# Zeudon/sound-event-localization-detection

Hardware: AMD Instinct MI355X
Metric: training clips/sec (4ch FOA 60s@24kHz) (higher is better)
Workload: dtype bf16; 1 GPU; crnn FOA 4-ch 60s clips, bs=32 windows (BASELINE configs[1]); parallelism=dp1

## Files before the change

sound-event-localization-detection_amd/csrc/conv3x3_image.h:

```cpp
#pragma once

#include <hip/hip_runtime.h>

namespace seld {
namespace conv3x3 {

typedef __attribute__((ext_vector_type(8))) __bf16 bf16x8;
typedef __attribute__((ext_vector_type(4))) short s16x4;
typedef __attribute__((ext_vector_type(8))) short s16x8;
typedef __attribute__((ext_vector_type(4))) float f32x4;
typedef __attribute__((address_space(3))) s16x4 lds_s16x4;

constexpr int kThreads = 256;
constexpr int kChannels = 64;
constexpr int kPitch = 80;

template <int F, int P>
struct Image {
  static_assert(F == 8 || F == 16 || F == 32, "frequency bins: 8, 16 or 32");
  static_assert(P % F == 0, "a chunk is whole time rows");
  static constexpr int TC = P / F;
  static constexpr int kRows = (TC + 2) * (F + 2);
  static constexpr int kLoads = (kRows * 8 + kThreads - 1) / kThreads;
};

template <int F>
__device__ __forceinline__ int image_row(int pos) {
  return (pos / F + 1) * (F + 2) + pos % F + 1;
}

template <int F>
__device__ __forceinline__ constexpr int tap_shift(int tap) {
  return (tap / 3 - 1) * (F + 2) + (tap % 3 - 1);
}

template <int F, int P>
__device__ __forceinline__ uint4 image_piece(const unsigned short* __restrict__ src, long clip_row, int t0, int T,
                                             int C, int c0, int piece) {
  const int r = piece >> 3, ch = piece & 7;
  const int tr = r / (F + 2), f = r - tr * (F + 2) - 1, t = t0 - 1 + tr;
  uint4 v = make_uint4(0u, 0u, 0u, 0u);
  if (r < Image<F, P>::kRows && t >= 0 && t < T && f >= 0 && f < F)
    v = *reinterpret_cast<const uint4*>(src + ((clip_row + t) * F + f) * C + c0 + ch * 8);
  return v;
}

__device__ __forceinline__ s16x4 tr_read(const unsigned short* base, int offset_shorts) {
  return __builtin_amdgcn_ds_read_tr16_b64_v4i16((lds_s16x4*)(base + offset_shorts));
}

__device__ __forceinline__ bf16x8 join(s16x4 lo, s16x4 hi) {
  const s16x8 v = __builtin_shufflevector(lo, hi, 0, 1, 2, 3, 4, 5, 6, 7);
  return __builtin_bit_cast(bf16x8, v);
}

}
}
```

sound-event-localization-detection_amd/csrc/conv3x3_loop.h:

```cpp
#pragma once

#include <hip/hip_bf16.h>

#include "conv3x3_image.h"

namespace seld {
namespace conv3x3 {

constexpr int kLoopP = 256;
constexpr int kLoopKc = kChannels;

template <int F, int NT, bool kFwd>
struct LoopGeom {
  static_assert(NT == 64 || NT == 128, "result channels per workgroup: 64 or 128");
  using Img = Image<F, kLoopP>;
  static constexpr int kWPitch = kFwd ? kPitch : NT + 16;
  static constexpr int kWRows = kFwd ? NT : kLoopKc;
  static constexpr int kWLoads = kLoopKc * NT / 8 / kThreads;
  static constexpr int kNTiles = NT / 32;
  static constexpr int kImgBatch = (Img::kLoads + 1) / 2;
  static constexpr int kImgShorts = Img::kRows * kPitch;
  static constexpr int kLdsShorts = kImgShorts + kWRows * kWPitch;
  static_assert(2 * kLdsShorts * 2 <= 160 * 1024, "two workgroups per CU");
};

template <int kCtrl>
__device__ __forceinline__ float dpp_add(float v) {
  return v + __builtin_bit_cast(float, __builtin_amdgcn_update_dpp(0, __builtin_bit_cast(int, v), kCtrl, 0xf, 0xf, false));
}
__device__ __forceinline__ float row16_sum(float v) {
  v = dpp_add<0xB1>(v);
  v = dpp_add<0x4E>(v);
  v = dpp_add<0x141>(v);
  return dpp_add<0x140>(v);
}

template <int F, int NT, bool kFwd, bool kStats>
__device__ __forceinline__ void conv3x3_loop(const unsigned short* __restrict__ src, const unsigned short* __restrict__ w,
                                             int T, int Cn, int Ck, int chunks_per_clip,
                                             unsigned short* __restrict__ dst, float* __restrict__ partials) {
  static_assert(kFwd || !kStats, "the statistics epilogue belongs to the forward direction");
  using G = LoopGeom<F, NT, kFwd>;
  __shared__ __attribute__((aligned(16))) unsigned short lds[G::kLdsShorts];
  unsigned short* const limg = lds;
  unsigned short* const lw = lds + G::kImgShorts;

  const int tid = threadIdx.x, lane = tid & 63, wave = tid >> 6;
  const int wm = wave >> 1, wn = wave & 1;
  const int chunk = blockIdx.x, n0 = blockIdx.y * NT;
  const int b = chunk / chunks_per_clip, t0 = (chunk - b * chunks_per_clip) * G::Img::TC;
  const long clip_row = static_cast<long>(b) * T;

  f32x4 acc[8][G::kNTiles];
#pragma unroll
  for (int m = 0; m < 8; ++m)
#pragma unroll
    for (int n = 0; n < G::kNTiles; ++n) acc[m][n] = f32x4{0.0f, 0.0f, 0.0f, 0.0f};

  const int g = lane >> 4, q = (lane >> 2) & 3, p = lane & 3, l15 = lane & 15;
  const int w_off = kFwd ? (wn * (NT / 2) + l15) * G::kWPitch + 8 * g
                         : (4 * g + q) * G::kWPitch + wn * (NT / 2) + 4 * p;
  const int d_off = image_row<F>(wm * 128 + l15) * kPitch + 8 * g;
  auto d_rows = [](int m) { return image_row<F>(16 * m) - image_row<F>(0); };

  static_assert(G::kWLoads == 2 || G::kWLoads == 4, "weight pieces per thread");
  uint4 rw0, rw1, rw2 = make_uint4(0u, 0u, 0u, 0u), rw3 = rw2;
  auto w_piece = [&](int stage, int i) {
    const int kc = stage / 9, tap = stage - kc * 9;
    const int piece = tid + i * kThreads;
    if constexpr (kFwd) {
      const int row = piece >> 3, ch = piece & 7;
      return *reinterpret_cast<const uint4*>(w + (static_cast<long>(n0 + row) * 9 + tap) * Ck + kc * kLoopKc + ch * 8);
    } else {
      const int row = piece / (NT / 8), ch = piece % (NT / 8);
      return *reinterpret_cast<const uint4*>(w + (static_cast<long>(kc * kLoopKc + row) * 9 + tap) * Cn + n0 + ch * 8);
    }
  };
  auto load_w = [&](int stage) {
    rw0 = w_piece(stage, 0);
    rw1 = w_piece(stage, 1);
    if constexpr (G::kWLoads == 4) {
      rw2 = w_piece(stage, 2);
      rw3 = w_piece(stage, 3);
    }
  };
  auto w_slot = [&](int i) {
    const int piece = tid + i * kThreads;
    if constexpr (kFwd) return reinterpret_cast<uint4*>(lw + (piece >> 3) * G::kWPitch + (piece & 7) * 8);
    else return reinterpret_cast<uint4*>(lw + piece / (NT / 8) * G::kWPitch + piece % (NT / 8) * 8);
  };

  const int stages = Ck / kLoopKc * 9;
  load_w(0);
  for (int stage = 0; stage < stages; ++stage) {
    const int kc = stage / 9, tap = stage - kc * 9;
    uint4 rimg[G::kImgBatch];
    auto load_img = [&](int first) {
#pragma unroll
      for (int i = 0; i < G::kImgBatch; ++i)
        rimg[i] = image_piece<F, kLoopP>(src, clip_row, t0, T, Ck, kc * kLoopKc, tid + (first + i) * kThreads);
    };
    auto store_img = [&](int first) {
#pragma unroll
      for (int i = 0; i < G::kImgBatch; ++i) {
        const int piece = tid + (first + i) * kThreads, ch = piece & 7;
        if constexpr (kFwd) {
          if (piece < G::Img::kRows * 8) *reinterpret_cast<uint4*>(limg + (piece >> 3) * kPitch + ch * 8) = rimg[i];
        } else {
          unsigned short* const slot = limg + (piece >> 3) * kPitch + (ch >> 2) * 32 + 16 * (ch & 1) + 4 * ((ch >> 1) & 1);
          if (piece < G::Img::kRows * 8) {
            *reinterpret_cast<uint2*>(slot) = make_uint2(rimg[i].x, rimg[i].y);
            *reinterpret_cast<uint2*>(slot + 8) = make_uint2(rimg[i].z, rimg[i].w);
          }
        }
      }
    };
    if (tap == 0) load_img(0);
    __syncthreads();
    *w_slot(0) = rw0;
    *w_slot(1) = rw1;
    if constexpr (G::kWLoads == 4) {
      *w_slot(2) = rw2;
      *w_slot(3) = rw3;
    }
    if (tap == 0) {
      store_img(0);
      load_img(G::kImgBatch);
      store_img(G::kImgBatch);
    }
    __syncthreads();
    load_w(min(stage + 1, stages - 1));

    const int shift = (kFwd ? tap_shift<F>(tap) : -tap_shift<F>(tap)) * kPitch;
#pragma unroll
    for (int ks = 0; ks < kLoopKc / 32; ++ks) {
      bf16x8 wf[G::kNTiles];
#pragma unroll
      for (int n = 0; n < G::kNTiles; ++n) {
        if constexpr (kFwd)
          wf[n] = *reinterpret_cast<const bf16x8*>(lw + w_off + n * 16 * G::kWPitch + ks * 32);
        else
          wf[n] = join(tr_read(lw, w_off + ks * 32 * G::kWPitch + n * 16),
                       tr_read(lw, w_off + (ks * 32 + 16) * G::kWPitch + n * 16));
      }
#pragma unroll
      for (int m = 0; m < 8; ++m) {
        const bf16x8 df = *reinterpret_cast<const bf16x8*>(limg + d_off + d_rows(m) * kPitch + shift + ks * 32);
#pragma unroll
        for (int n = 0; n < G::kNTiles; ++n)
          acc[m][n] = __builtin_amdgcn_mfma_f32_16x16x32_bf16(wf[n], df, acc[m][n], 0, 0, 0);
      }
    }
  }

  const int rows_left = (T - t0) * F;
  unsigned short* const out = dst + ((clip_row + t0) * F) * Cn + n0 + wn * (NT / 2) + 4 * g;
#pragma unroll
  for (int m = 0; m < 8; ++m) {
    const int pos = wm * 128 + m * 16 + l15;
    if (pos >= rows_left) continue;
#pragma unroll
    for (int n = 0; n < G::kNTiles; ++n) {
      const f32x4 v = acc[m][n];
      const unsigned lo = static_cast<unsigned>(__bfloat16_as_ushort(__float2bfloat16(v[0]))) |
                          (static_cast<unsigned>(__bfloat16_as_ushort(__float2bfloat16(v[1]))) << 16);
      const unsigned hi = static_cast<unsigned>(__bfloat16_as_ushort(__float2bfloat16(v[2]))) |
                          (static_cast<unsigned>(__bfloat16_as_ushort(__float2bfloat16(v[3]))) << 16);
      *reinterpret_cast<uint2*>(out + static_cast<long>(pos) * Cn + n * 16) = make_uint2(lo, hi);
    }
  }

  if constexpr (kStats) {
    float* const red = reinterpret_cast<float*>(lds);
    __syncthreads();
#pragma unroll
    for (int n = 0; n < G::kNTiles; ++n)
#pragma unroll
      for (int j = 0; j < 4; ++j) {
        float r[8], s[8];
#pragma unroll
        for (int m = 0; m < 8; ++m) {
          const float v = __uint_as_float(static_cast<unsigned>(__bfloat16_as_ushort(__float2bfloat16(acc[m][n][j]))) << 16);
          r[m] = wm * 128 + m * 16 + l15 < rows_left ? v : 0.0f;
          s[m] = r[m] * r[m];
        }
        const float s1 = row16_sum(((r[0] + r[1]) + (r[2] + r[3])) + ((r[4] + r[5]) + (r[6] + r[7])));
        const float s2 = row16_sum(((s[0] + s[1]) + (s[2] + s[3])) + ((s[4] + s[5]) + (s[6] + s[7])));
        if (l15 == 0) {
          const int c = wn * (NT / 2) + n * 16 + 4 * g + j;
          red[(wm * 2 + 0) * NT + c] = s1;
          red[(wm * 2 + 1) * NT + c] = s2;
        }
      }
    __syncthreads();
    if (tid < 2 * NT) {
      const int stat = tid / NT, c = tid - stat * NT;
      partials[(static_cast<long>(stat) * gridDim.x + chunk) * Cn + n0 + c] = red[stat * NT + c] + red[(2 + stat) * NT + c];
    }
  }
}

}
}
```

sound-event-localization-detection_amd/csrc/convdgrad.hip:

```cpp
#include <hip/hip_bf16.h>

#include "conv3x3_loop.h"
#include "seld_common.h"

namespace seld {

namespace {

using namespace conv3x3;

constexpr int kDgP = kLoopP;
constexpr int kDgKc = kLoopKc;

template <int F, int NT>
__global__ __launch_bounds__(kThreads, 2) void conv3x3_dgrad_kernel(
    const unsigned short* __restrict__ dy, const unsigned short* __restrict__ w, int T, int Cin, int Cout,
    int chunks_per_clip, unsigned short* __restrict__ dx) {
  conv3x3_loop<F, NT, false, false>(dy, w, T, Cin, Cout, chunks_per_clip, dx, nullptr);
}

bool dgrad_supported(int64_t F, int64_t Cin, int64_t Cout) {
  return (F == 8 || F == 16 || F == 32) && Cin > 0 && Cout > 0 && Cin % 64 == 0 && Cout % kDgKc == 0;
}

template <int F>
void launch_dgrad(const unsigned short* dy, const unsigned short* w, int B, int T, int Cin, int Cout,
                  unsigned short* dx, hipStream_t stream) {
  constexpr int tc = kDgP / F;
  const int chunks_per_clip = (T + tc - 1) / tc;
  const unsigned chunks = static_cast<unsigned>(B * chunks_per_clip);
  if (Cin % 128 == 0)
    hipLaunchKernelGGL((conv3x3_dgrad_kernel<F, 128>), dim3(chunks, static_cast<unsigned>(Cin / 128)), dim3(kThreads),
                       0, stream, dy, w, T, Cin, Cout, chunks_per_clip, dx);
  else
    hipLaunchKernelGGL((conv3x3_dgrad_kernel<F, 64>), dim3(chunks, static_cast<unsigned>(Cin / 64)), dim3(kThreads), 0,
                       stream, dy, w, T, Cin, Cout, chunks_per_clip, dx);
}

}

}

extern "C" {

int seld_conv3x3_dgrad_supported(int64_t F, int64_t Cin, int64_t Cout) {
  return seld::dgrad_supported(F, Cin, Cout) ? 1 : 0;
}

int seld_conv3x3_dgrad(const void* dy, const void* w, int64_t B, int64_t T, int64_t F, int64_t Cin, int64_t Cout,
                       void* dx, void* stream_) {
  using namespace seld;
  const DeviceState* st = current_state();
  if (!st) return kErrNotInitialised;
  if (!dy || !w || !dx || B <= 0 || T <= 0) return fail(kErrInvalidArgument, "seld_conv3x3_dgrad: bad argument");
  if (!dgrad_supported(F, Cin, Cout))
    return fail(kErrUnsupported, "seld_conv3x3_dgrad: F in {8, 16, 32} and channel counts % 64 == 0 required");
  if (B * ((T + kDgP / F - 1) / (kDgP / F)) > 0x7fffffffLL || B * T > 0x7fffffffLL)
    return fail(kErrUnsupported, "seld_conv3x3_dgrad: too many positions");
  if (((reinterpret_cast<uintptr_t>(dy) | reinterpret_cast<uintptr_t>(w) | reinterpret_cast<uintptr_t>(dx)) & 15) != 0)
    return fail(kErrInvalidArgument, "seld_conv3x3_dgrad: 16-byte aligned tensors required");
  hipStream_t stream = static_cast<hipStream_t>(stream_);
  const unsigned short* ds = static_cast<const unsigned short*>(dy);
  const unsigned short* ws = static_cast<const unsigned short*>(w);
  unsigned short* xs = static_cast<unsigned short*>(dx);
  const int b = static_cast<int>(B), t = static_cast<int>(T), ci = static_cast<int>(Cin), co = static_cast<int>(Cout);
  switch (F) {
    case 8: launch_dgrad<8>(ds, ws, b, t, ci, co, xs, stream); break;
    case 16: launch_dgrad<16>(ds, ws, b, t, ci, co, xs, stream); break;
    default: launch_dgrad<32>(ds, ws, b, t, ci, co, xs, stream); break;
  }
  SELD_HIP_TRY(hipGetLastError());
  return kOk;
}

}
```

sound-event-localization-detection_amd/csrc/convfwd.hip:

```cpp
#include <hip/hip_bf16.h>

#include "conv3x3_loop.h"
#include "seld_common.h"

namespace seld {

namespace {

using namespace conv3x3;

template <int F, int NT, bool kStats>
__global__ __launch_bounds__(kThreads, 2) void conv3x3_fwd_kernel(
    const unsigned short* __restrict__ x, const unsigned short* __restrict__ w, int T, int Cin, int Cout,
    int chunks_per_clip, unsigned short* __restrict__ y, float* __restrict__ partials) {
  conv3x3_loop<F, NT, true, kStats>(x, w, T, Cout, Cin, chunks_per_clip, y, partials);
}

bool fwd_supported(int64_t F, int64_t Cin, int64_t Cout) {
  return (F == 8 || F == 16 || F == 32) && Cin > 0 && Cout > 0 && Cin % kLoopKc == 0 && Cout % 64 == 0;
}

int64_t fwd_chunks(int64_t B, int64_t T, int64_t F) {
  const int64_t tc = kLoopP / F;
  return B * ((T + tc - 1) / tc);
}

template <int F, int NT>
void launch_fwd_tile(const unsigned short* x, const unsigned short* w, int T, int Cin, int Cout, int chunks_per_clip,
                     unsigned chunks, unsigned short* y, float* partials, hipStream_t stream) {
  const dim3 grid(chunks, static_cast<unsigned>(Cout / NT));
  if (partials)
    hipLaunchKernelGGL((conv3x3_fwd_kernel<F, NT, true>), grid, dim3(kThreads), 0, stream, x, w, T, Cin, Cout,
                       chunks_per_clip, y, partials);
  else
    hipLaunchKernelGGL((conv3x3_fwd_kernel<F, NT, false>), grid, dim3(kThreads), 0, stream, x, w, T, Cin, Cout,
                       chunks_per_clip, y, partials);
}

template <int F>
void launch_fwd(const unsigned short* x, const unsigned short* w, int B, int T, int Cin, int Cout, unsigned short* y,
                float* partials, hipStream_t stream) {
  constexpr int tc = kLoopP / F;
  const int chunks_per_clip = (T + tc - 1) / tc;
  const unsigned chunks = static_cast<unsigned>(B * chunks_per_clip);
  if (Cout % 128 == 0) launch_fwd_tile<F, 128>(x, w, T, Cin, Cout, chunks_per_clip, chunks, y, partials, stream);
  else launch_fwd_tile<F, 64>(x, w, T, Cin, Cout, chunks_per_clip, chunks, y, partials, stream);
}

}

}

extern "C" {

int seld_conv3x3_forward_supported(int64_t F, int64_t Cin, int64_t Cout) {
  return seld::fwd_supported(F, Cin, Cout) ? 1 : 0;
}

int64_t seld_conv3x3_forward_chunks(int64_t B, int64_t T, int64_t F) {
  if (!(F == 8 || F == 16 || F == 32) || B <= 0 || T <= 0) return 0;
  return seld::fwd_chunks(B, T, F);
}

int seld_conv3x3_forward(const void* x, const void* w, int64_t B, int64_t T, int64_t F, int64_t Cin, int64_t Cout,
                         void* y, float* partials, void* stream_) {
  using namespace seld;
  const DeviceState* st = current_state();
  if (!st) return kErrNotInitialised;
  if (!x || !w || !y || B <= 0 || T <= 0) return fail(kErrInvalidArgument, "seld_conv3x3_forward: bad argument");
  if (!fwd_supported(F, Cin, Cout))
    return fail(kErrUnsupported, "seld_conv3x3_forward: F in {8, 16, 32} and channel counts % 64 == 0 required");
  if (fwd_chunks(B, T, F) > 0x7fffffffLL || B * T > 0x7fffffffLL)
    return fail(kErrUnsupported, "seld_conv3x3_forward: too many positions");
  if (((reinterpret_cast<uintptr_t>(x) | reinterpret_cast<uintptr_t>(w) | reinterpret_cast<uintptr_t>(y)) & 15) != 0)
    return fail(kErrInvalidArgument, "seld_conv3x3_forward: 16-byte aligned tensors required");
  hipStream_t stream = static_cast<hipStream_t>(stream_);
  const unsigned short* xs = static_cast<const unsigned short*>(x);
  const unsigned short* ws = static_cast<const unsigned short*>(w);
  unsigned short* ys = static_cast<unsigned short*>(y);
  const int b = static_cast<int>(B), t = static_cast<int>(T), ci = static_cast<int>(Cin), co = static_cast<int>(Cout);
  switch (F) {
    case 8: launch_fwd<8>(xs, ws, b, t, ci, co, ys, partials, stream); break;
    case 16: launch_fwd<16>(xs, ws, b, t, ci, co, ys, partials, stream); break;
    default: launch_fwd<32>(xs, ws, b, t, ci, co, ys, partials, stream); break;
  }
  SELD_HIP_TRY(hipGetLastError());
  return kOk;
}

}
```

Before: 172.0 clips/s.

## Software-pipeline LDS reads in conv3x3 loop and widen output stores

Restructures the inner MFMA loop of the shared conv3x3 forward and dgrad kernel into a flat step sequence with a rotating lookahead buffer of image fragments and staggered weight fragment reads. Scheduling barriers pin the order so LDS latency overlaps MFMA work. Weight loads now use a precomputed 32-bit per-thread offset off a per-stage base pointer, and the channel limit guard added to the support checks keeps that offset from overflowing. The epilogue uses permlane16_swap to pair rows and emit 16-byte stores instead of 8-byte ones. In exchange, register pressure rises and the scheduler has less freedom.

```diff
diff --git a/sound-event-localization-detection_amd/csrc/conv3x3_image.h b/sound-event-localization-detection_amd/csrc/conv3x3_image.h
--- a/sound-event-localization-detection_amd/csrc/conv3x3_image.h
+++ b/sound-event-localization-detection_amd/csrc/conv3x3_image.h
@@ -9,6 +9,8 @@
 typedef __attribute__((ext_vector_type(4))) short s16x4;
 typedef __attribute__((ext_vector_type(8))) short s16x8;
 typedef __attribute__((ext_vector_type(4))) float f32x4;
+typedef __attribute__((ext_vector_type(4))) unsigned u32x4;
+typedef __attribute__((ext_vector_type(2))) unsigned u32x2;
 typedef __attribute__((address_space(3))) s16x4 lds_s16x4;
 
 constexpr int kThreads = 256;
diff --git a/sound-event-localization-detection_amd/csrc/conv3x3_loop.h b/sound-event-localization-detection_amd/csrc/conv3x3_loop.h
--- a/sound-event-localization-detection_amd/csrc/conv3x3_loop.h
+++ b/sound-event-localization-detection_amd/csrc/conv3x3_loop.h
@@ -9,6 +9,7 @@
 
 constexpr int kLoopP = 256;
 constexpr int kLoopKc = kChannels;
+constexpr int kLoopMaxChannels = 1 << 20;
 
 template <int F, int NT, bool kFwd>
 struct LoopGeom {
@@ -19,6 +20,7 @@
   static constexpr int kWLoads = kLoopKc * NT / 8 / kThreads;
   static constexpr int kNTiles = NT / 32;
   static constexpr int kImgBatch = (Img::kLoads + 1) / 2;
+  static constexpr int kAhead = NT == 128 ? 2 : 4;
   static constexpr int kImgShorts = Img::kRows * kPitch;
   static constexpr int kLdsShorts = kImgShorts + kWRows * kWPitch;
   static_assert(2 * kLdsShorts * 2 <= 160 * 1024, "two workgroups per CU");
@@ -64,30 +66,31 @@
   auto d_rows = [](int m) { return image_row<F>(16 * m) - image_row<F>(0); };
 
   static_assert(G::kWLoads == 2 || G::kWLoads == 4, "weight pieces per thread");
-  uint4 rw0, rw1, rw2 = make_uint4(0u, 0u, 0u, 0u), rw3 = rw2;
-  auto w_piece = [&](int stage, int i) {
+  constexpr int kWPieceRows = kFwd ? kThreads / 8 : kThreads / (NT / 8);
+  const long w_row = 9L * (kFwd ? Ck : Cn);
+  const unsigned w_voff = kFwd ? ((tid >> 3) * 9 * Ck + (tid & 7) * 8) * 2u
+                               : ((tid / (NT / 8)) * 9 * Cn + (tid % (NT / 8)) * 8) * 2u;
+  u32x4 rw0, rw1, rw2 = u32x4{0u, 0u, 0u, 0u}, rw3 = rw2;
+  auto w_piece = [&](const unsigned short* base, int i, unsigned voff) {
+    return *reinterpret_cast<const u32x4*>(reinterpret_cast<const char*>(base + i * kWPieceRows * w_row) + voff);
+  };
+  auto load_w = [&](int stage) {
+    unsigned voff = w_voff;
+    asm volatile("" : "+v"(voff));
     const int kc = stage / 9, tap = stage - kc * 9;
-    const int piece = tid + i * kThreads;
-    if constexpr (kFwd) {
-      const int row = piece >> 3, ch = piece & 7;
-      return *reinterpret_cast<const uint4*>(w + (static_cast<long>(n0 + row) * 9 + tap) * Ck + kc * kLoopKc + ch * 8);
-    } else {
-      const int row = piece / (NT / 8), ch = piece % (NT / 8);
-      return *reinterpret_cast<const uint4*>(w + (static_cast<long>(kc * kLoopKc + row) * 9 + tap) * Cn + n0 + ch * 8);
-    }
-  };
-  auto load_w = [&](int stage) {
-    rw0 = w_piece(stage, 0);
-    rw1 = w_piece(stage, 1);
+    const unsigned short* const base = kFwd ? w + (n0 * 9L + tap) * Ck + kc * kLoopKc
+                                            : w + (kc * kLoopKc * 9L + tap) * Cn + n0;
+    rw0 = w_piece(base, 0, voff);
+    rw1 = w_piece(base, 1, voff);
     if constexpr (G::kWLoads == 4) {
-      rw2 = w_piece(stage, 2);
-      rw3 = w_piece(stage, 3);
+      rw2 = w_piece(base, 2, voff);
+      rw3 = w_piece(base, 3, voff);
     }
   };
   auto w_slot = [&](int i) {
     const int piece = tid + i * kThreads;
-    if constexpr (kFwd) return reinterpret_cast<uint4*>(lw + (piece >> 3) * G::kWPitch + (piece & 7) * 8);
-    else return reinterpret_cast<uint4*>(lw + piece / (NT / 8) * G::kWPitch + piece % (NT / 8) * 8);
+    if constexpr (kFwd) return reinterpret_cast<u32x4*>(lw + (piece >> 3) * G::kWPitch + (piece & 7) * 8);
+    else return reinterpret_cast<u32x4*>(lw + piece / (NT / 8) * G::kWPitch + piece % (NT / 8) * 8);
   };
 
   const int stages = Ck / kLoopKc * 9;
@@ -96,9 +99,11 @@
     const int kc = stage / 9, tap = stage - kc * 9;
     uint4 rimg[G::kImgBatch];
     auto load_img = [&](int first) {
+      int t = tid;
+      asm volatile("" : "+v"(t));
 #pragma unroll
       for (int i = 0; i < G::kImgBatch; ++i)
-        rimg[i] = image_piece<F, kLoopP>(src, clip_row, t0, T, Ck, kc * kLoopKc, tid + (first + i) * kThreads);
+        rimg[i] = image_piece<F, kLoopP>(src, clip_row, t0, T, Ck, kc * kLoopKc, t + (first + i) * kThreads);
     };
     auto store_img = [&](int first) {
 #pragma unroll
@@ -130,43 +135,57 @@
     }
     __syncthreads();
     load_w(min(stage + 1, stages - 1));
+    __builtin_amdgcn_sched_barrier(0);
 
     const int shift = (kFwd ? tap_shift<F>(tap) : -tap_shift<F>(tap)) * kPitch;
-#pragma unroll
-    for (int ks = 0; ks < kLoopKc / 32; ++ks) {
-      bf16x8 wf[G::kNTiles];
-#pragma unroll
-      for (int n = 0; n < G::kNTiles; ++n) {
-        if constexpr (kFwd)
-          wf[n] = *reinterpret_cast<const bf16x8*>(lw + w_off + n * 16 * G::kWPitch + ks * 32);
-        else
-          wf[n] = join(tr_read(lw, w_off + ks * 32 * G::kWPitch + n * 16),
-                       tr_read(lw, w_off + (ks * 32 + 16) * G::kWPitch + n * 16));
-      }
-#pragma unroll
-      for (int m = 0; m < 8; ++m) {
-        const bf16x8 df = *reinterpret_cast<const bf16x8*>(limg + d_off + d_rows(m) * kPitch + shift + ks * 32);
-#pragma unroll
-        for (int n = 0; n < G::kNTiles; ++n)
-          acc[m][n] = __builtin_amdgcn_mfma_f32_16x16x32_bf16(wf[n], df, acc[m][n], 0, 0, 0);
-      }
-    }
+    constexpr int kSteps = 8 * (kLoopKc / 32);
+    constexpr int kAhead = G::kAhead;
+    auto read_w = [&](int ks, int n) {
+      if constexpr (kFwd)
+        return *reinterpret_cast<const bf16x8*>(lw + w_off + n * 16 * G::kWPitch + ks * 32);
+      else
+        return join(tr_read(lw, w_off + ks * 32 * G::kWPitch + n * 16),
+                    tr_read(lw, w_off + (ks * 32 + 16) * G::kWPitch + n * 16));
+    };
+    auto read_d = [&](int step) {
+      return *reinterpret_cast<const bf16x8*>(limg + d_off + d_rows(step & 7) * kPitch + shift + (step >> 3) * 32);
+    };
+    bf16x8 wf[kLoopKc / 32][G::kNTiles], df[kAhead + 1];
+#pragma unroll
+    for (int n = 0; n < G::kNTiles; ++n) wf[0][n] = read_w(0, n);
+#pragma unroll
+    for (int a = 0; a < kAhead; ++a) df[a] = read_d(a);
+    __builtin_amdgcn_sched_barrier(0);
+#pragma unroll
+    for (int step = 0; step < kSteps; ++step) {
+      const int ks = step >> 3, m = step & 7;
+      if (step + kAhead < kSteps) df[(step + kAhead) % (kAhead + 1)] = read_d(step + kAhead);
+      if (ks + 1 < kLoopKc / 32 && m < G::kNTiles) wf[ks + 1][m] = read_w(ks + 1, m);
+#pragma unroll
+      for (int n = 0; n < G::kNTiles; ++n)
+        acc[m][n] = __builtin_amdgcn_mfma_f32_16x16x32_bf16(wf[ks][n], df[step % (kAhead + 1)], acc[m][n], 0, 0, 0);
+      __builtin_amdgcn_sched_barrier(0);
+    }
+    asm volatile("" : "+v"(rw0), "+v"(rw1));
+    if constexpr (G::kWLoads == 4) asm volatile("" : "+v"(rw2), "+v"(rw3));
   }
 
   const int rows_left = (T - t0) * F;
-  unsigned short* const out = dst + ((clip_row + t0) * F) * Cn + n0 + wn * (NT / 2) + 4 * g;
-#pragma unroll
-  for (int m = 0; m < 8; ++m) {
-    const int pos = wm * 128 + m * 16 + l15;
-    if (pos >= rows_left) continue;
+  unsigned short* const out = dst + ((clip_row + t0) * F) * Cn + n0 + wn * (NT / 2) + 4 * (g & ~1);
+  auto pack = [](float a, float c) {
+    return static_cast<unsigned>(__bfloat16_as_ushort(__float2bfloat16(a))) |
+           (static_cast<unsigned>(__bfloat16_as_ushort(__float2bfloat16(c))) << 16);
+  };
+#pragma unroll
+  for (int k = 0; k < 4; ++k) {
+    const int pos = wm * 128 + (2 * k + (g & 1)) * 16 + l15;
 #pragma unroll
     for (int n = 0; n < G::kNTiles; ++n) {
-      const f32x4 v = acc[m][n];
-      const unsigned lo = static_cast<unsigned>(__bfloat16_as_ushort(__float2bfloat16(v[0]))) |
-                          (static_cast<unsigned>(__bfloat16_as_ushort(__float2bfloat16(v[1]))) << 16);
-      const unsigned hi = static_cast<unsigned>(__bfloat16_as_ushort(__float2bfloat16(v[2]))) |
-                          (static_cast<unsigned>(__bfloat16_as_ushort(__float2bfloat16(v[3]))) << 16);
-      *reinterpret_cast<uint2*>(out + static_cast<long>(pos) * Cn + n * 16) = make_uint2(lo, hi);
+      const f32x4 v0 = acc[2 * k][n], v1 = acc[2 * k + 1][n];
+      const u32x2 lo = __builtin_amdgcn_permlane16_swap(pack(v0[0], v0[1]), pack(v1[0], v1[1]), false, false);
+      const u32x2 hi = __builtin_amdgcn_permlane16_swap(pack(v0[2], v0[3]), pack(v1[2], v1[3]), false, false);
+      if (pos < rows_left)
+        *reinterpret_cast<u32x4*>(out + static_cast<long>(pos) * Cn + n * 16) = u32x4{lo[0], hi[0], lo[1], hi[1]};
     }
   }
 
diff --git a/sound-event-localization-detection_amd/csrc/convdgrad.hip b/sound-event-localization-detection_amd/csrc/convdgrad.hip
--- a/sound-event-localization-detection_amd/csrc/convdgrad.hip
+++ b/sound-event-localization-detection_amd/csrc/convdgrad.hip
@@ -20,7 +20,8 @@
 }
 
 bool dgrad_supported(int64_t F, int64_t Cin, int64_t Cout) {
-  return (F == 8 || F == 16 || F == 32) && Cin > 0 && Cout > 0 && Cin % 64 == 0 && Cout % kDgKc == 0;
+  return (F == 8 || F == 16 || F == 32) && Cin > 0 && Cout > 0 && Cin % 64 == 0 && Cout % kDgKc == 0 &&
+         Cin <= kLoopMaxChannels && Cout <= kLoopMaxChannels;
 }
 
 template <int F>
diff --git a/sound-event-localization-detection_amd/csrc/convfwd.hip b/sound-event-localization-detection_amd/csrc/convfwd.hip
--- a/sound-event-localization-detection_amd/csrc/convfwd.hip
+++ b/sound-event-localization-detection_amd/csrc/convfwd.hip
@@ -17,7 +17,8 @@
 }
 
 bool fwd_supported(int64_t F, int64_t Cin, int64_t Cout) {
-  return (F == 8 || F == 16 || F == 32) && Cin > 0 && Cout > 0 && Cin % kLoopKc == 0 && Cout % 64 == 0;
+  return (F == 8 || F == 16 || F == 32) && Cin > 0 && Cout > 0 && Cin % kLoopKc == 0 && Cout % 64 == 0 &&
+         Cin <= kLoopMaxChannels && Cout <= kLoopMaxChannels;
 }
 
 int64_t fwd_chunks(int64_t B, int64_t T, int64_t F) {
```

Result: faster. 176.1 clips/s, median of 6 (+2.4%).
